# Tonmoy1321/Multimodal-DeepFake-Detection

Hardware: AMD Instinct MI355X
Metric: clips/sec (node) XceptionLSTMV 16x299x299 bf16 train (higher is better)
Workload: dtype bf16; 1 GPU; XceptionLSTMV(hidden=128) unfrozen-backbone train step, 16 clips/GPU x 16 frames x 3x299x299, BCE + clip 1.0 + Adam; global_batch=16, frames=16, size=299, mode=unfrozen, optimizer=clip 1.0 + Adam, xcp FusedAdamClip, parallelism=dp1, execution=eager launches

## Files before the change

include/xcp.h:

```cpp
#ifndef XCP_H_
#define XCP_H_

#ifdef __cplusplus
extern "C" {
#endif

typedef void* xcp_stream_t;

#define XCP_OK 0
#define XCP_EINVAL 1001
#define XCP_EUNSUPPORTED 1002
#define XCP_F32 0
#define XCP_BF16 1
#define XCP_ACT_NONE 0
#define XCP_ACT_RELU 1
#define XCP_ACT_BNRELU 2

int xcp_gemm_nt(int dtype, const void* A, long lda, const void* B, long ldb, void* C, long ldc, int M, int N, int K,
                float* stats, int gmode, int gH, int gW, int gOH, int gOW, int gS, int gC, int tile, xcp_stream_t stream);
int xcp_gemm_nt_stat_rows(int M);

int xcp_gemm_tn_rows_per_split(int dtype, int gmode, int M, int N, int K, int tile);
int xcp_gemm_tn(int dtype, const void* G, long ldg, const void* X, long ldx, float* P, int M, int N, int K, int S,
                int rows_per_split, int gmode, int gH, int gW, int gOH, int gOW, int gS, int gC, int tile,
                xcp_stream_t stream);

int xcp_unit_bwd_rows_per_split(int dtype, int M, int CO, int CI);
int xcp_unit_bwd(int dtype, const void* G, const void* Y, const float* alpha, const float* bcoef, const float* delta,
                 const void* Wt, const void* X, void* dD, float* P, int M, int CO, int CI, int S, int rows_per_split,
                 xcp_stream_t stream);

int xcp_dw_fwd(int dtype, int act, const void* X, void* Y, const float* Wt, const float* scale, const float* shift, int N,
               int H, int W, int C, xcp_stream_t stream);
int xcp_sep_fwd_parts(int dtype, int N, int H, int W, int CIN, int COUT);
int xcp_sep_fwd(int dtype, int act, const void* X, const float* scale, const float* shift, const float* dwt, const void* pw,
                void* D, void* Y, float* part, int N, int H, int W, int CIN, int COUT, xcp_stream_t stream);
int xcp_dw_bwd_chunks(int N, int H, int W, int C);
int xcp_dw_bwd(int dtype, int act, const void* dY, const void* X, const float* Wt, const float* scale, const float* shift,
               const void* dRes, const void* dSkip, int sOH, int sOW, int sS, int skip_pre, void* dX, float* dWpart,
               float* bnpart, const float* bmean, const float* binvstd, int N, int H, int W, int C,
               xcp_stream_t stream);
int xcp_dw_bwd_resbn(int dtype, int act, const void* dY, const void* X, const float* Wt, const float* scale,
                     const float* shift, const void* dRes, void* dX, float* dWpart, float* bnpart, const float* bmean,
                     const float* binvstd, const void* Yb, int N, int H, int W, int C, xcp_stream_t stream);

int xcp_colreduce_f32(const float* in, int S, long L, long ld, float* out, int G, int accumulate, xcp_stream_t stream);
int xcp_colreduce_multi(const long long* jobs, int njobs, xcp_stream_t stream);
int xcp_colreduce_groups(int S, long L);
int xcp_chanred_parts(long rows, int C);
int xcp_row_stats(int dtype, const void* X, long rows, int C, float* part, xcp_stream_t stream);
int xcp_bn_bwd_reduce(int dtype, const void* dZ, const void* Y, const float* mean, const float* invstd,
                      const float* ms, const float* mt, long rows, int C, float* part, xcp_stream_t stream);
int xcp_bn_finalize_part(const float* part, int R, int C, int CP, double count, const float* gamma, const float* beta,
                         float* rmean, float* rvar, float momentum, float eps, float* mean_o, float* invstd_o,
                         float* scale_o, float* shift_o, xcp_stream_t stream);
#define XCP_FIN_ACCUMULATE 1
#define XCP_FIN_NARROW 2
#define XCP_FIN_FROZEN 4
int xcp_bn_bwd_finalize_part(const float* part, int R, int C, int CP, double count, const float* gamma,
                             const float* mean, const float* invstd, float* alpha, float* bcoef, float* delta,
                             float* dgamma, float* dbeta, int flags, xcp_stream_t stream);
int xcp_bn_finalize(const double* part2, int G, int C, int CP, double count, const float* gamma, const float* beta,
                    float* rmean, float* rvar, float momentum, float eps, int train, float* mean, float* invstd,
                    float* scale, float* shift, xcp_stream_t stream);
int xcp_bn_act(int dtype, const void* X, void* Y, const float* scale, const float* shift, int relu, long rows, int C,
               xcp_stream_t stream);
int xcp_bn_act_strided(int dtype, const void* X, void* Y, const float* scale, const float* shift, int relu, int N, int H,
                       int W, int OH, int OW, int S, int C, xcp_stream_t stream);
int xcp_bn_bwd_apply(int dtype, const void* dZ, const void* Y, void* dY, const float* alpha, const float* bcoef,
// ... 102 lines not shown
```

multimodal-deepfake-detection_amd/xcp/_lib.py:

```python
import ctypes
import os

_HERE = os.path.dirname(os.path.abspath(__file__))
LIB_PATH = DEFAULT_LIB_PATH = os.path.join(_HERE, "libxcp.so")
_REPO = os.path.dirname(os.path.dirname(_HERE))
_OVERRIDE = os.environ.get("XCP_LIB_PATH")
if _OVERRIDE:
    _real = os.path.realpath(_OVERRIDE)
    if os.path.commonpath([_real, os.path.realpath(_REPO)]) != os.path.realpath(_REPO):
        raise ImportError(f"XCP_LIB_PATH={_OVERRIDE} is outside the repository ({_REPO}); "
                          "only in-tree A/B builds may replace libxcp.so")
    LIB_PATH = _real
MISSING = []

P = ctypes.c_void_p
I = ctypes.c_int
L = ctypes.c_long
F = ctypes.c_float
D = ctypes.c_double

SIGNATURES = {
    "xcp_gemm_nt": [I, P, L, P, L, P, L, I, I, I, P, I, I, I, I, I, I, I, I, P],
    "xcp_gemm_nt_stat_rows": [I],
    "xcp_gemm_tn_rows_per_split": [I, I, I, I, I, I],
    "xcp_gemm_tn": [I, P, L, P, L, P, I, I, I, I, I, I, I, I, I, I, I, I, I, P],
    "xcp_unit_bwd_rows_per_split": [I, I, I, I],
    "xcp_unit_bwd": [I, P, P, P, P, P, P, P, P, P, I, I, I, I, I, P],
    "xcp_dw_fwd": [I, I, P, P, P, P, P, I, I, I, I, P],
    "xcp_sep_fwd_parts": [I, I, I, I, I, I],
    "xcp_sep_fwd": [I, I, P, P, P, P, P, P, P, P, I, I, I, I, I, P],
    "xcp_dw_bwd_chunks": [I, I, I, I],
    "xcp_dw_bwd": [I, I, P, P, P, P, P, P, P, I, I, I, I, P, P, P, P, P, I, I, I, I, P],
    "xcp_dw_bwd_resbn": [I, I, P, P, P, P, P, P, P, P, P, P, P, P, I, I, I, I, P],
    "xcp_colreduce_f32": [P, I, L, L, P, I, I, P],
    "xcp_colreduce_groups": [I, L],
    "xcp_colreduce_multi": [P, I, P],
    "xcp_chanred_parts": [L, I],
    "xcp_row_stats": [I, P, L, I, P, P],
    "xcp_bn_bwd_reduce": [I, P, P, P, P, P, P, L, I, P, P],
    "xcp_bn_finalize_part": [P, I, I, I, D, P, P, P, P, F, F, P, P, P, P, P],
    "xcp_bn_bwd_finalize_part": [P, I, I, I, D, P, P, P, P, P, P, P, P, I, P],
    "xcp_bn_finalize": [P, I, I, I, D, P, P, P, P, F, F, I, P, P, P, P, P],
    "xcp_bn_act": [I, P, P, P, P, I, L, I, P],
    "xcp_bn_act_strided": [I, P, P, P, P, I, I, I, I, I, I, I, I, P],
    "xcp_bn_bwd_apply": [I, P, P, P, P, P, P, P, P, L, I, P],
    "xcp_relu_bwd": [I, P, P, L, I, P],
    "xcp_tail_fwd": [I, P, P, P, I, P, P, P, P, P, I, I, I, I, P],
    "xcp_maxpool_bwd": [I, P, P, P, I, I, I, I, P],
    "xcp_maxpool_bwd_bnred_parts": [I, I, I, I],
    "xcp_maxpool_bwd_bnred": [I, P, P, P, P, P, P, I, I, I, I, P, P],
    "xcp_avgpool_fwd": [I, P, P, P, P, I, I, I, P],
    "xcp_avgpool_bwd": [I, P, P, P, P, P, I, I, I, P],
    "xcp_conv1_fwd": [I, P, P, P, I, I, I, P],
    "xcp_conv1_fwd_parts": [I, I, I],
    "xcp_conv1_fwd_stats": [I, P, P, P, P, I, I, I, P],
    "xcp_conv1_wgrad_parts": [I, I, I],
    "xcp_conv1_wgrad": [I, P, P, P, I, I, I, P],
    "xcp_conv1_wgrad_fused": [I, I, I],
    "xcp_conv1_wgrad_bn": [I, P, P, P, P, P, P, P, P, P, I, I, I, P],
    "xcp_conv1_dgrad": [I, P, P, P, I, I, I, P],
    "xcp_conv1_dgrad_bn": [I, P, P, P, P, P, P, P, P, P, I, I, I, P],
    "xcp_permute3": [I, P, P, I, I, I, I, I, I, P],
    "xcp_permute3_blocks": [I, I, I, I, I, I, L, L],
    "xcp_permute3_batch": [P, I, I, P],
    "xcp_frames_u8_to_f32": [P, P, P, I, I, I, I, P],
    "xcp_resize_bilinear": [P, P, I, I, I, I, I, P],
    "xcp_frames_prep": [P, P, P, I, I, I, I, I, I, I, I, P],
    "xcp_opt_sumsq": [P, I, P, F, P, P],
    "xcp_opt_adam": [P, I, P, F, F, F, F, F, F, F, P],
    "xcp_opt_adam_dev": [P, I, P, F, D, D, F, F, P, P],
    "xcp_opt_sumsq_amp": [P, I, P, F, P, P, P],
    "xcp_opt_adam_amp": [P, I, P, F, F, F, F, F, F, F, F, P, P, P],
    "xcp_opt_adam_amp_dev": [P, I, P, F, D, D, F, F, F, P, P, P, P],
    "xcp_opt_average": [P, I, P, D, P, P],
    "xcp_conv3x3_parts": [I, I, I, I],
    "xcp_conv3x3": [I, P, P, P, P, I, I, I, P, P, P],
    "xcp_conv3x3_wgrad_parts": [I, I, I],
    "xcp_conv3x3_wgrad": [P, P, P, I, I, I, P, P, P],
    "xcp_arcface_fwd": [P, P, P, P, I, I, I, F, F, P],
    "xcp_arcface_bwd": [P, P, P, P, P, P, I, I, I, F, F, P],
    "xcp_focal_ce": [P, P, P, F, P, P, P, I, I, P],
    "xcp_lstm_needs_whhT": [I, I, I],
    "xcp_lstm_fwd": [P, P, P, P, P, P, P, P, P, P, P, I, I, I, I, P],
    "xcp_lstm_bwd": [P, P, P, P, P, P, P, P, I, I, I, I, P],
    "xcp_lstm_sync_error": [],
    "xcp_lstm_varlen_needs_whhT": [I, I, I],
    "xcp_lstm_fwd_varlen": [P, P, P, P, P, P, P, P, P, P, P, P, I, I, I, I, P],
    "xcp_lstm_bwd_varlen": [P, P, P, P, P, P, P, P, P, I, I, I, I, P],
    "xcp_clock_probe": [P, I, I, P],
    "xcp_stream_copy": [P, P, L, P],
    "xcp_comm_proxy": [P, P, L, I, ctypes.c_longlong, P, P],
    "xcp_stamp": [P, P],
}

SIZE_QUERIES = {"xcp_permute3_blocks", "xcp_sep_fwd_parts", "xcp_gemm_tn_rows_per_split", "xcp_gemm_nt_stat_rows", "xcp_dw_bwd_chunks", "xcp_chanred_parts",
                "xcp_colreduce_groups", "xcp_unit_bwd_rows_per_split",
                "xcp_conv1_wgrad_parts", "xcp_conv1_wgrad_fused", "xcp_conv1_fwd_parts", "xcp_lstm_needs_whhT", "xcp_conv3x3_parts", "xcp_conv3x3_wgrad_parts",
                "xcp_maxpool_bwd_bnred_parts", "xcp_lstm_sync_error", "xcp_lstm_varlen_needs_whhT"}

_lib = None


class XcpError(RuntimeError):
    pass


def load():
    global _lib
    if _lib is not None:
        return _lib
    import torch
    if not os.path.exists(LIB_PATH):
        raise XcpError(f"HIP library {LIB_PATH} is missing; run `python -m xcp.build` (hipcc, gfx950). "
                       "There is no CPU fallback for the product path.")
    lib = ctypes.CDLL(LIB_PATH)
    for name, argtypes in SIGNATURES.items():
        if LIB_PATH != DEFAULT_LIB_PATH and not hasattr(lib, name):
            MISSING.append(name)
            continue
        fn = getattr(lib, name)
        fn.argtypes = argtypes
        fn.restype = ctypes.c_int
    if LIB_PATH != DEFAULT_LIB_PATH:
        import sys
        print(f"xcp: XCP_LIB_PATH override {LIB_PATH}; entry points it lacks: {MISSING or 'none'}",
              file=sys.stderr)
    _lib = lib
    return lib
# ... 14 lines not shown
```

multimodal-deepfake-detection_amd/xcp/csrc/sepfwd.hip:

```cpp
#include "common.h"

namespace {

constexpr int SP_WMAX = 152;
constexpr int SP_WMAX1 = 78;
constexpr int SP_HALF = 80;
constexpr int SP_SEG = 5;
constexpr unsigned SP_OOB = 0x80000000u;
constexpr int SP_REC = 0x7fffffff;
constexpr int SP_DW3 = 0x00020000;

typedef int i32x4 __attribute__((ext_vector_type(4)));
typedef int i32x2 __attribute__((ext_vector_type(2)));
typedef unsigned u32x4 __attribute__((ext_vector_type(4)));
typedef float f2 __attribute__((ext_vector_type(2)));


XCP_DEV u32x4 sp_bload(__amdgpu_buffer_rsrc_t r, int off) {
  u32x4 v;
  asm volatile("buffer_load_dwordx4 %0, %1, %2, 0 offen" : "=v"(v) : "v"(off), "s"(r) : "memory");
  return v;
}

template <int N>
// ... 10 lines not shown
  const bf16* pw;
  bf16* D;
  bf16* Y;
  float* part;
  int N, H, W;
  int nbands, bandH;
};

XCP_DEV void sp_vm_wait(int n) {
  switch (n < 0 ? 0 : n > 63 ? 63 : n) {
#define SP_VMW(k) case k: asm volatile("s_waitcnt vmcnt(" #k ")" ::: "memory"); break;
    SP_VMW(0) SP_VMW(1) SP_VMW(2) SP_VMW(3) SP_VMW(4) SP_VMW(5) SP_VMW(6) SP_VMW(7)
    SP_VMW(8) SP_VMW(9) SP_VMW(10) SP_VMW(11) SP_VMW(12) SP_VMW(13) SP_VMW(14) SP_VMW(15)
    SP_VMW(16) SP_VMW(17) SP_VMW(18) SP_VMW(19) SP_VMW(20) SP_VMW(21) SP_VMW(22) SP_VMW(23)
    SP_VMW(24) SP_VMW(25) SP_VMW(26) SP_VMW(27) SP_VMW(28) SP_VMW(29) SP_VMW(30) SP_VMW(31)
    SP_VMW(32) SP_VMW(33) SP_VMW(34) SP_VMW(35) SP_VMW(36) SP_VMW(37) SP_VMW(38) SP_VMW(39)
#undef SP_VMW
    default: asm volatile("s_waitcnt vmcnt(40)" ::: "memory"); break;
  }
}

XCP_DEV void sp_barrier() {
  asm volatile("s_waitcnt lgkmcnt(0)" ::: "memory");
  __builtin_amdgcn_s_barrier();
  asm volatile("" ::: "memory");
}

XCP_DEV float sp_lo(unsigned u) { return __uint_as_float(u << 16); }
XCP_DEV float sp_hi(unsigned u) { return __uint_as_float(u & 0xffff0000u); }
XCP_DEV unsigned sp_pack(float a, float b) { return pk_bf16(a, b); }

template <int ACT, int CIN, int COUT, int NHALF>
__global__ __launch_bounds__(512) void sep_fwd_kernel(SepArgs a) {
  constexpr int SP_RPX = (NHALF == 2 ? SP_WMAX : SP_WMAX1) + 2;
  constexpr int NB = COUT / 128;
  constexpr int YC = COUT / 8;
  constexpr int S = CIN / 32;
  constexpr int CH = CIN / 8;
  constexpr int PB = CIN * 2;
  constexpr int RB = SP_RPX * PB;
  constexpr int DP = PB + 16;
  constexpr int KL = (SP_RPX * CH + 511) / 512;
  constexpr int KD = (SP_HALF * CH + 511) / 512;
  constexpr int LPS = CIN / 2;
  constexpr int SPW = 64 / LPS;
  constexpr int NPASS = (SP_HALF / SP_SEG) / (8 * SPW);
  constexpr int YP = COUT * 2 + 16;
  constexpr int KY = (SP_HALF * YC + 511) / 512;
  constexpr bool YSHARE = YP == DP;
  constexpr int NST = NHALF * (KD + KY);
  static_assert(NST + KL <= 39, "counted wait exceeds sp_vm_wait's range");
  __shared__ __attribute__((aligned(16))) char rows[3 * RB];
  __shared__ __attribute__((aligned(16))) char dt[SP_HALF * DP];
  __shared__ __attribute__((aligned(16))) char yown[YSHARE ? 16 : SP_HALF * YP];
  char* const yt = YSHARE ? dt : yown;
  __shared__ __attribute__((aligned(16))) float stap[9][CIN];
  __shared__ __attribute__((aligned(16))) float sprm[2][CIN];

  const int tid = threadIdx.x, lane = tid & 63, w = __builtin_amdgcn_readfirstlane(tid >> 6);
  const int fr = lane & 15, fg = lane >> 4;
  const int H = a.H, W = a.W;
  const int nch = (W + 2) * CH;
  const __amdgpu_buffer_rsrc_t rD = __builtin_amdgcn_make_buffer_rsrc(a.D, (short)0, SP_REC, SP_DW3);
  const __amdgpu_buffer_rsrc_t rY = __builtin_amdgcn_make_buffer_rsrc(a.Y, (short)0, SP_REC, SP_DW3);

  bf16x8 wf[NB][S];
#pragma unroll
  for (int j = 0; j < NB; ++j)
#pragma unroll
    for (int s = 0; s < S; ++s)
      wf[j][s] = *reinterpret_cast<const bf16x8*>(a.pw + (long)((w + 8 * j) * 16 + fr) * CIN + s * 32 + fg * 8);
  for (int c = tid; c < 9 * CIN; c += 512) stap[c / CIN][c % CIN] = a.dwt[c];
  for (int c = tid; c < CIN; c += 512) {
    sprm[0][c] = ACT == ACT_BNRELU ? a.scale[c] : 1.f;
    sprm[1][c] = ACT == ACT_BNRELU ? a.shift[c] : 0.f;
  }
  __syncthreads();
  const int ch = 2 * (lane % LPS);
  const int q = tid % CH;
  f2 s1[4], s2[4];
#pragma unroll
  for (int r = 0; r < 4; ++r) s1[r] = s2[r] = f2{0.f, 0.f};

  u32x4 rga[KL], rgb[KL];
  int loff[KL];
#pragma unroll
  for (int k = 0; k < KL; ++k) {
    const int c = tid + 512 * k;
    const int px = c / CH;
    loff[k] = c < nch && px >= 1 && px <= W ? ((px - 1) * CIN + q * 8) * 2 : (int)SP_OOB;
  }
  auto load_row = [&](u32x4 (&rg)[KL], int n, int hh) {
    const bool rok = hh >= 0 && hh < H;
    const __amdgpu_buffer_rsrc_t rs = __builtin_amdgcn_make_buffer_rsrc(
        const_cast<bf16*>(a.X + ((long)n * H + (rok ? hh : 0)) * W * CIN), (short)0, rok ? SP_REC : 0, SP_DW3);
#pragma unroll
    for (int k = 0; k < KL; ++k) rg[k] = sp_bload(rs, loff[k]);
  };
  auto store_row = [&](u32x4 (&rg)[KL], int hh) {
    sp_fence(rg);
    char* slot = rows + ((hh + 3) % 3) * RB;
#pragma unroll
    for (int k = 0; k < KL; ++k) {
      const int c = tid + 512 * k;
      if (c >= nch) continue;
      const int px = c / CH;
      uint4 u = make_uint4(rg[k][0], rg[k][1], rg[k][2], rg[k][3]);
      if constexpr (ACT != ACT_NONE) {
        if (hh >= 0 && hh < H && px >= 1 && px <= W) {
          unsigned v[4] = {u.x, u.y, u.z, u.w};
#pragma unroll
          for (int e = 0; e < 4; ++e) {
            f2 x = f2{sp_lo(v[e]), sp_hi(v[e])};
            if constexpr (ACT == ACT_BNRELU)
              x = __builtin_elementwise_fma(x, *reinterpret_cast<const f2*>(&sprm[0][q * 8 + 2 * e]),
                                            *reinterpret_cast<const f2*>(&sprm[1][q * 8 + 2 * e]));
            x = __builtin_elementwise_max(x, f2{0.f, 0.f});
            v[e] = sp_pack(x[0], x[1]);
          }
          u = make_uint4(v[0], v[1], v[2], v[3]);
        }
      }
      *reinterpret_cast<uint4*>(slot + px * PB + q * 16) = u;
    }
  };

  const int tiles = a.N * a.nbands;
  for (int tile = xcd_remap(blockIdx.x, gridDim.x); tile < tiles; tile += gridDim.x) {
    const int n = tile / a.nbands, band = tile % a.nbands;
    const int r0 = band * a.bandH, r1 = min(H, r0 + a.bandH);
    sp_barrier();
    for (int hh = r0 - 1; hh <= r0 + 1; ++hh) {
      load_row(rga, n, hh);
      sp_vm_wait(0);
      store_row(rga, hh);
    }
    load_row(rga, n, r0 + 2);
    load_row(rgb, n, r0 + 3);
    sp_barrier();
    auto row = [&](int h, u32x4 (&rg)[KL]) {
      const long prow = ((long)n * H + h) * W;
      const char* rw0 = rows + ((h + 2) % 3) * RB;
      const char* rw1 = rows + ((h + 3) % 3) * RB;
      const char* rw2 = rows + ((h + 4) % 3) * RB;
#pragma unroll
      for (int hf = 0; hf < NHALF; ++hf) {
        f32x4 acc[5][NB];
#pragma unroll
        for (int b = 0; b < 5; ++b)
#pragma unroll
          for (int j = 0; j < NB; ++j) acc[b][j] = f32x4{0.f, 0.f, 0.f, 0.f};
#pragma unroll 1
        for (int p = 0; p < NPASS; ++p) {
          const int seg = p * 8 * SPW + w * SPW + lane / LPS;
          const int xl = seg * SP_SEG;
          const int x0 = hf * SP_HALF + xl;
          f2 tp[9];
#pragma unroll
          for (int t = 0; t < 9; ++t) tp[t] = *reinterpret_cast<const f2*>(&stap[t][ch]);
          f2 win[3][SP_SEG + 2];
#pragma unroll
          for (int k = 0; k < SP_SEG + 2; ++k) {
            const int off = min(x0 + k, W + 1) * PB + ch * 2;
            const unsigned u0 = *reinterpret_cast<const unsigned*>(rw0 + off);
            const unsigned u1 = *reinterpret_cast<const unsigned*>(rw1 + off);
            const unsigned u2 = *reinterpret_cast<const unsigned*>(rw2 + off);
            win[0][k] = f2{sp_lo(u0), sp_hi(u0)};
            win[1][k] = f2{sp_lo(u1), sp_hi(u1)};
            win[2][k] = f2{sp_lo(u2), sp_hi(u2)};
          }
#pragma unroll
          for (int jj = 0; jj < SP_SEG; ++jj) {
            f2 d = f2{0.f, 0.f};
#pragma unroll
            for (int ky = 0; ky < 3; ++ky)
#pragma unroll
              for (int kx = 0; kx < 3; ++kx) d = __builtin_elementwise_fma(win[ky][jj + kx], tp[ky * 3 + kx], d);
            *reinterpret_cast<unsigned*>(dt + (xl + jj) * DP + ch * 2) = x0 + jj < W ? sp_pack(d[0], d[1]) : 0u;
          }
        }
        sp_barrier();
#pragma unroll
        for (int b = 0; b < 5; ++b)
#pragma unroll
          for (int s = 0; s < S; ++s) {
            const bf16x8 ad = *reinterpret_cast<const bf16x8*>(dt + (b * 16 + fr) * DP + (s * 32 + fg * 8) * 2);
#pragma unroll
            for (int j = 0; j < NB; ++j) acc[b][j] = __builtin_amdgcn_mfma_f32_16x16x32_bf16(wf[j][s], ad, acc[b][j], 0, 0, 0);
          }
#pragma unroll
        for (int k = 0; k < KD; ++k) {
          const int c = tid + 512 * k;
          const int pl = min(c / CH, SP_HALF - 1), qq = c % CH;
          const int px = hf * SP_HALF + pl;
          const bool ok = c < SP_HALF * CH && px < W;
          const uint4 v = *reinterpret_cast<const uint4*>(dt + pl * DP + qq * 16);
          const unsigned off = ok ? (unsigned)(((prow + px) * CIN + qq * 8) * 2) : SP_OOB;
          __builtin_amdgcn_raw_buffer_store_b128(__builtin_bit_cast(i32x4, v), rD, (int)off, 0, 0);
        }
        if constexpr (YSHARE) sp_barrier();
#pragma unroll
        for (int b = 0; b < 5; ++b)
#pragma unroll
          for (int j = 0; j < NB; ++j)
            *reinterpret_cast<uint2*>(yt + (b * 16 + fr) * YP + ((w + 8 * j) * 16 + 4 * fg) * 2) =
                make_uint2(sp_pack(acc[b][j][0], acc[b][j][1]), sp_pack(acc[b][j][2], acc[b][j][3]));
        sp_barrier();
#pragma unroll
        for (int k = 0; k < KY; ++k) {
          const int c = tid + 512 * k;
          const int pl = min(c / YC, SP_HALF - 1), qq = c % YC;
          const int px = hf * SP_HALF + pl;
          const bool ok = c < SP_HALF * YC && px < W;
          const uint4 v = *reinterpret_cast<const uint4*>(yt + pl * YP + qq * 16);
          const unsigned off = ok ? (unsigned)(((prow + px) * COUT + qq * 8) * 2) : SP_OOB;
          __builtin_amdgcn_raw_buffer_store_b128(__builtin_bit_cast(i32x4, v), rY, (int)off, 0, 0);
          if (ok) {
            const unsigned u4[4] = {v.x, v.y, v.z, v.w};
#pragma unroll
            for (int r = 0; r < 4; ++r) {
              const f2 y = f2{sp_lo(u4[r]), sp_hi(u4[r])};
              s1[r] += y;
              s2[r] = __builtin_elementwise_fma(y, y, s2[r]);
            }
          }
        }
        sp_barrier();
      }
      sp_vm_wait(NST + KL);
      store_row(rg, h + 2);
      load_row(rg, n, h + 4);
      sp_barrier();
    };
    for (int h = r0; h < r1; h += 2) {
      row(h, rga);
      if (h + 1 < r1) row(h + 1, rgb);
    }
    sp_vm_wait(0);
  }
  sp_vm_wait(0);
  if (a.part) {
    float t[2][8];
#pragma unroll
    for (int r = 0; r < 4; ++r)
#pragma unroll
      for (int e = 0; e < 2; ++e) {
        t[0][2 * r + e] = s1[r][e];
        t[1][2 * r + e] = s2[r][e];
      }
#pragma unroll
    for (int m = 0; m < 2; ++m)
#pragma unroll
      for (int e = 0; e < 8; ++e) {
        if constexpr (YC == 16) t[m][e] += __shfl_xor(t[m][e], 16, 64);
        t[m][e] += __shfl_xor(t[m][e], 32, 64);
      }
    sp_barrier();
// ... 3 lines not shown
      for (int m = 0; m < 2; ++m)
#pragma unroll
        for (int e = 0; e < 8; ++e) red[(w * 2 + m) * COUT + lane * 8 + e] = t[m][e];
    sp_barrier();
    for (int i = tid; i < 2 * COUT; i += 512) {
      float v = 0.f;
#pragma unroll
      for (int ww = 0; ww < 8; ++ww) v += red[ww * 2 * COUT + i];
      a.part[(long)blockIdx.x * 2 * COUT + i] = v;
    }
  }
}

int sp_cus() {
  static const int v = [] {
    int dev = 0, n = 0;
    if (hipGetDevice(&dev) != hipSuccess || hipDeviceGetAttribute(&n, hipDeviceAttributeMultiprocessorCount, dev) != hipSuccess)
      n = 0;
    return n > 0 ? n : 256;
  }();
  return v;
}

void sp_bands(int N, int H, int& nb, int& bandH) {
  const int cus = sp_cus();
  nb = N >= cus ? 1 : (cus + N - 1) / N;
  const int maxb = H >= 16 ? H / 8 : 1;
  if (nb > maxb) nb = maxb;
  if (nb < 1) nb = 1;
  bandH = (H + nb - 1) / nb;
  nb = (H + bandH - 1) / bandH;
}

}

extern "C" {

int xcp_sep_fwd_parts(int dtype, int N, int H, int W, int CIN, int COUT) {
  const bool shape = (COUT == 128 && (CIN == 64 || CIN == 128) && W <= SP_WMAX) ||
                     (COUT == 256 && CIN == 128 && W <= SP_WMAX1);
  if (dtype != XCP_BF16 || !shape || W < 1 || N <= 0 || H <= 0) return 0;
  const long pix = (long)N * H * W;
  if (pix * CIN * 2 > 0x7fffffffL || pix * COUT * 2 > 0x7fffffffL) return 0;
  int nb, bh;
  sp_bands(N, H, nb, bh);
  const long tiles = (long)N * nb;
  return (int)(tiles < sp_cus() ? tiles : sp_cus());
}

int xcp_sep_fwd(int dtype, int act, const void* X, const float* scale, const float* shift, const float* dwt, const void* pw,
                void* D, void* Y, float* part, int N, int H, int W, int CIN, int COUT, hipStream_t stream) {
  const int grid = xcp_sep_fwd_parts(dtype, N, H, W, CIN, COUT);
  if (grid <= 0) return XCP_EUNSUPPORTED;
  if (act < ACT_NONE || act > ACT_BNRELU || (act == ACT_BNRELU && (!scale || !shift))) return XCP_EINVAL;
  SepArgs a{(const bf16*)X, scale, shift, dwt, (const bf16*)pw, (bf16*)D, (bf16*)Y, part, N, H, W, 1, H};
  sp_bands(N, H, a.nbands, a.bandH);
#define SP_LAUNCH(A, C, O, NH) hipLaunchKernelGGL((sep_fwd_kernel<A, C, O, NH>), dim3(grid), dim3(512), 0, stream, a)
#define SP_ACTS(C, O, NH)                          \
  if (act == ACT_NONE) SP_LAUNCH(ACT_NONE, C, O, NH); \
  else if (act == ACT_RELU) SP_LAUNCH(ACT_RELU, C, O, NH); \
  else SP_LAUNCH(ACT_BNRELU, C, O, NH);
  if (COUT == 256) {
    SP_ACTS(128, 256, 1)
  } else if (CIN == 64) {
    SP_ACTS(64, 128, 2)
  } else {
    SP_ACTS(128, 128, 2)
  }
#undef SP_ACTS
#undef SP_LAUNCH
  return (int)hipGetLastError();
}

}
```

multimodal-deepfake-detection_amd/xcp/engine.py:

```python
import contextlib
import os
import math

import torch
import torch.nn as nn

from . import ops
from .ops import ACT_BNRELU, ACT_NONE, ACT_RELU


def _bn_ref(m):
    return {"weight": m.weight, "bias": m.bias, "running_mean": m.running_mean, "running_var": m.running_var,
            "eps": m.eps, "momentum": m.momentum, "track": m.track_running_stats, "module": m}


class _Unit:

    def __init__(self, sep, bn, relu, name, bn_name):
        self.sep, self.bn, self.relu, self.name, self.bn_name = sep, bn, relu, name, bn_name
        self.cin = sep.conv1.in_channels
        self.cout = sep.pointwise.out_channels
        if sep.conv1.kernel_size != (3, 3) or sep.conv1.stride != (1, 1) or sep.conv1.padding != (1, 1):
            raise NotImplementedError("xcp engine supports the Xception 3x3/s1/p1 separable convs only")
        if sep.conv1.bias is not None or sep.pointwise.bias is not None:
# ... 34 lines not shown
        if self.pool and self.skip is None:
            raise NotImplementedError("xcp engine: a pooled block needs a conv skip")
        if self.skip is not None and self.stride != (2 if self.pool else 1):
            raise NotImplementedError("xcp engine: skip stride must match the pooling")
        self.cin = self.units[0].cin
        self.cout = self.units[-1].cout


class Stats:
    __slots__ = ("mean", "invstd", "scale", "shift")

    def __init__(self, C, dev):
        buf = torch.empty(4 * C, device=dev, dtype=torch.float32)
        self.mean, self.invstd, self.scale, self.shift = buf[:C], buf[C:2 * C], buf[2 * C:3 * C], buf[3 * C:]

    def __getitem__(self, k):
        return getattr(self, k)


WGRAD_SIDE_STREAM = os.environ.get("XCP_WGRAD_STREAM", "1") != "0"
FUSED_UNIT_BWD = os.environ.get("XCP_FUSED_UNIT_BWD", "1") != "0"
STEM_FUSED = os.environ.get("XCP_STEM_FUSED", "1") != "0"
RESBN = os.environ.get("XCP_RESBN", "0") == "1"
STEM_WGRAD_SIDE = WGRAD_SIDE_STREAM and os.environ.get("XCP_STEM_WGRAD_SIDE", "1") != "0"
SIDE_PRIO_LOW = os.environ.get("XCP_SIDE_PRIO", "") == "low"
STEM_BN1_FIRST = os.environ.get("XCP_STEM_BN1_FIRST", "1") != "0"
CONV1_BN_FUSED = os.environ.get("XCP_CONV1_BN_FUSED", "1") != "0"
STEM_WGRAD_EARLY = os.environ.get("XCP_STEM_WGRAD_EARLY", "1") != "0"
STEM_FIN_NARROW = os.environ.get("XCP_STEM_FIN_NARROW", "1") != "0"
CONV1_STATS_FUSED = os.environ.get("XCP_CONV1_STATS_FUSED", "1") != "0"
DW_REDUCE_SIDE = WGRAD_SIDE_STREAM and os.environ.get("XCP_DW_REDUCE_SIDE", "1") != "0"
REDUCE_BATCH = os.environ.get("XCP_REDUCE_BATCH", "1") != "0"
SEP_FUSED = os.environ.get("XCP_SEP_FUSED", "1") != "0"
SEP_MIN_W = {128: 0, 256: 0} if os.environ.get("XCP_SEP_NARROW", "0") == "1" else {128: 120, 256: 64}
CONV2_ACT_ON_LOAD = os.environ.get("XCP_CONV2_ACTIN", "1") != "0"
WGRAD_FIRST = os.environ.get("XCP_WGRAD_FIRST", "0") == "1"
WGRAD_DEFER = os.environ.get("XCP_WGRAD_DEFER", "0") == "1"
SKIP_WGRAD_LATE = os.environ.get("XCP_SKIP_WGRAD_LATE", "0") == "1"
NT_TILE = int(os.environ.get("XCP_NT_TILE", "4" if os.environ.get("XCP_NT_ONESHOT", "0") == "1" else "0"))
_pad = os.environ.get("XCP_PAD_728", "736")
PAD_PITCH = {} if _pad == "0" else {728: int(_pad)}
if PAD_PITCH and (PAD_PITCH[728] < 728 or PAD_PITCH[728] % 8):
    raise ValueError("XCP_PAD_728 must be 0 or a multiple of 8 >= 728")


def pc(c):
    return PAD_PITCH.get(c, c)


class XceptionEngine:
    def __init__(self, model, dtype=torch.bfloat16):
        if dtype not in (torch.float32, torch.bfloat16):
            raise ValueError("xcp engine dtype must be float32 (parity) or bfloat16")
        self.model = model
        self.dtype = dtype
        self.blocks = [_Block(getattr(model, f"block{i}"), f"block{i}") for i in range(1, 13)]
        self.exit_units = [_Unit(model.conv3, model.bn3, False, "conv3", "bn3"),
                           _Unit(model.conv4, model.bn4, True, "conv4", "bn4")]
        c1, c2 = model.conv1, model.conv2
        if (c1.in_channels, c1.out_channels, c1.kernel_size, c1.stride, c1.padding) != (3, 32, (3, 3), (2, 2), (0, 0)):
            raise NotImplementedError("xcp engine: Xception stem conv1 must be 3->32 3x3 s2 p0")
        if (c2.in_channels, c2.out_channels, c2.kernel_size, c2.stride, c2.padding) != (32, 64, (3, 3), (1, 1), (0, 0)):
            raise NotImplementedError("xcp engine: Xception stem conv2 must be 32->64 3x3 s1 p0")
        self.bn_named = [(n, m) for n, m in model.named_modules() if isinstance(m, nn.BatchNorm2d)]
        self.bn_modules = [m for _, m in self.bn_named]
        self._pack_key = None
# ... 195 lines not shown
            H, W, rest = OH2, OW2, self.blocks
        for b in rest:
            xc, H, W, bs = self._block_fwd(b, xc, N, H, W, pk, train)
            S["blocks"].append(bs)
        M = N * H * W
        ex = []
        src, act, sc, sh = xc, ACT_NONE, None, None
        for u in self.exit_units:
            d = self._empty(M * pc(u.cin))
            ops.dw_fwd(act, src, d, pk[u.name + ".dw"], sc, sh, N, H, W, pc(u.cin))
            y, st = self._pw(d, pk[u.name + ".pw"], M, u.cout, u.cin, train, u.bn)
            ex.append({"src": src, "act": act, "sc": sc, "sh": sh, "d": d, "y": y, "st": st})
            src, act, sc, sh = y, ACT_BNRELU, st.scale, st.shift
        feats = torch.empty(N, 2048, device=self.device, dtype=torch.float32)
        last = ex[-1]
        ops.avgpool_fwd(last["y"], last["st"].scale, last["st"].shift, feats, N, H * W, 2048)
        S.update(exit=ex, xH=H, xW=W, x12=xc)
        if train:
            nbt = [b.num_batches_tracked for b in self.bn_modules if b.num_batches_tracked is not None]
            if nbt:
                torch._foreach_add_(nbt, 1)
        return feats, S

    def _block_fwd(self, b, x_in, N, H, W, pk, train, pre_bn=None, skip_x=None):
        if pre_bn is not None and (b.skip is None or b.stride == 1 or b.units[0].relu):
            raise ValueError("pre_bn: only a block without a leading ReLU and with a strided skip conv")
        M = N * H * W
        units = []
        src, act, sc, sh = x_in, (ACT_RELU if b.units[0].relu else ACT_NONE), None, None
        if pre_bn is not None:
            act, sc, sh = ACT_BNRELU, pre_bn.scale, pre_bn.shift
        for u in b.units:
            d = self._empty(M * pc(u.cin))
            R = (ops.sep_fwd_parts(self.dtype, N, H, W, u.cin, u.cout)
                 if SEP_FUSED and train and pc(u.cin) == u.cin and pc(u.cout) == u.cout
                 and W >= SEP_MIN_W.get(u.cout, 1 << 30) else 0)
            if R > 0:
                y = self._empty(M * u.cout)
                part = self._empty(R * 2 * u.cout, torch.float32)
                ops.sep_fwd(act, src, sc, sh, pk[u.name + ".dw"], pk[u.name + ".pw"], d, y, part, N, H, W, u.cin, u.cout)
                st = self._bn_stats(part, R, u.cout, M, u.bn, True)
            else:
                ops.dw_fwd(act, src, d, pk[u.name + ".dw"], sc, sh, N, H, W, pc(u.cin))
                y, st = self._pw(d, pk[u.name + ".pw"], M, u.cout, u.cin, train, u.bn)
            units.append({"src": src, "act": act, "sc": sc, "sh": sh, "d": d, "y": y, "st": st})
            src, act, sc, sh = y, ACT_BNRELU, st.scale, st.shift
        if b.pool or b.stride != 1:
            OH, OW = (H - 1) // b.stride + 1, (W - 1) // b.stride + 1
        else:
            OH, OW = H, W
        Ms = N * OH * OW
        ys = sks = None
        if b.skip is not None and skip_x is not None:
            ys, sks = self._pw(skip_x, pk[b.name + ".skip"], Ms, b.cout, b.cin, train, b.skipbn, lda=pc(b.cin))
        elif b.skip is not None:
            ys, sks = self._pw(x_in, pk[b.name + ".skip"], Ms, b.cout, b.cin, train, b.skipbn, lda=pc(b.cin),
                               gather=(1, H, W, OH, OW, b.stride, 0) if b.stride != 1 else (0, 0, 0, 0, 0, 1, 0))
        out = self._empty(Ms * pc(b.cout))
        amax = torch.empty(Ms * pc(b.cout), device=self.device, dtype=torch.uint8) if b.pool else None
        st = units[-1]["st"]
        ops.tail_fwd(units[-1]["y"], st.scale, st.shift, b.pool, ys if ys is not None else x_in,
                     sks.scale if sks is not None else None, sks.shift if sks is not None else None, out, amax, N, H, W,
                     pc(b.cout))
        bs = {"x_in": x_in, "units": units, "ys": ys, "sks": sks, "amax": amax, "H": H, "W": W, "OH": OH, "OW": OW,
              "pre_bn": pre_bn, "skip_x": skip_x}
        return out, OH, OW, bs

    INPUT = "<frames>"

    def backward(self, S, dfeat, out=None, notify=None, need=None, input_grad=False):
        with ops.device_guard(dfeat):
            return self._backward(S, dfeat, out, notify, need, input_grad)

# ... 288 lines not shown
```

multimodal-deepfake-detection_amd/xcp/ops.py:

```python
import torch

from . import _lib

F32, BF16 = 0, 1
ACT_NONE, ACT_RELU, ACT_BNRELU = 0, 1, 2
DT = {torch.float32: F32, torch.bfloat16: BF16}


def _p(t):
    return 0 if t is None else t.data_ptr()


def stream():
    return torch.cuda.current_stream().cuda_stream


def device_guard(t):
    return torch.cuda.device(t.device)


class KernelTimer:

    def __init__(self, classes):
        self.classes = classes
# ... 121 lines not shown
                arr = (ctypes.c_longlong * len(vals))(*vals)
                _lib.call("xcp_colreduce_multi", ctypes.addressof(arr), len(chunk), stream())
        self.jobs = []


def weight_grad(G, X, M, N, K, out, gather=(0, 0, 0, 0, 0, 1, 0), ldg=None, ldx=None, tile=0, accumulate=False,
                batch=None):
    rps = _lib.call("xcp_gemm_tn_rows_per_split", DT[G.dtype], gather[0], M, N, K, tile)
    S = (M + rps - 1) // rps
    P = torch.empty(S * N * K, device=G.device, dtype=torch.float32)
    gemm_tn(G, X, P, M, N, K, S, rps, ldg=ldg, ldx=ldx, gather=gather, tile=tile)
    if batch is not None:
        batch.add(P, S, N * K, out, accumulate)
    else:
        reduce_slabs(P, S, N * K, out, accumulate)


def dw_fwd(act, X, Y, Wt, scale, shift, N, H, W, C):
    with _timed("dw_fwd", {"N": N, "H": H, "W": W, "C": C}):
        _lib.call("xcp_dw_fwd", DT[X.dtype], act, _p(X), _p(Y), _p(Wt), _p(scale), _p(shift), N, H, W, C, stream())


def sep_fwd_parts(dtype, N, H, W, cin, cout):
    return _lib.call("xcp_sep_fwd_parts", DT[dtype], N, H, W, cin, cout)


def sep_fwd(act, X, scale, shift, dwt, pw, D, Y, part, N, H, W, cin, cout):
    check_gpu(X, D, Y)
    with _timed("sep_fwd", {"N": N, "H": H, "W": W, "C": cin, "CO": cout}):
        _lib.call("xcp_sep_fwd", DT[X.dtype], act, _p(X), _p(scale), _p(shift), _p(dwt), _p(pw), _p(D), _p(Y), _p(part),
                  N, H, W, cin, cout, stream())


def dw_bwd(act, dY, X, Wt, scale, shift, dX, dW_out, N, H, W, C, dRes=None, dSkip=None, skip_geom=(0, 0, 1),
           bn_stats=None, accumulate=False, Cw=None, skip_pre=False, reduce_stream=None, keep=None, batch=None,
           res_bn_input=None):
    P = _lib.call("xcp_dw_bwd_chunks", N, H, W, C)
    part = torch.empty(P * C * 9, device=dY.device, dtype=torch.float32)
    bnpart = None
    if bn_stats is not None:
        bnpart = torch.empty(P * 2 * C, device=dY.device, dtype=torch.float32)
    if res_bn_input is not None:
        if dRes is None or dSkip is not None or bn_stats is None:
            raise ValueError("xcp.dw_bwd: res_bn_input needs dRes, no dSkip and the BN's bn_stats")
        _lib.call("xcp_dw_bwd_resbn", DT[dY.dtype], act, _p(dY), _p(X), _p(Wt), _p(scale), _p(shift), _p(dRes),
                  _p(dX), _p(part), _p(bnpart), _p(bn_stats["mean"]), _p(bn_stats["invstd"]), _p(res_bn_input),
                  N, H, W, C, stream())
    else:
        _lib.call("xcp_dw_bwd", DT[dY.dtype], act, _p(dY), _p(X), _p(Wt), _p(scale), _p(shift), _p(dRes), _p(dSkip),
                  skip_geom[0], skip_geom[1], skip_geom[2], int(skip_pre), _p(dX), _p(part), _p(bnpart),
                  _p(bn_stats["mean"]) if bn_stats is not None else 0,
                  _p(bn_stats["invstd"]) if bn_stats is not None else 0, N, H, W, C, stream())
    if dW_out is None:
        pass
    elif batch is not None:
        batch.add(part, P, (Cw or C) * 9, dW_out, accumulate, ld=C * 9)
        if keep is not None:
            keep.append(part)
    elif reduce_stream is None:
        reduce_slabs(part, P, (Cw or C) * 9, dW_out, accumulate, ld=C * 9)
    else:
        reduce_stream.wait_stream(torch.cuda.current_stream(dY.device))
        with torch.cuda.stream(reduce_stream):
            reduce_slabs(part, P, (Cw or C) * 9, dW_out, accumulate, ld=C * 9)
        if keep is not None:
            keep.append(part)
# ... 330 lines not shown
```

Measured before the change: 441.9 clips/s.

## Extend fused depthwise+pointwise separable forward kernel to 256->256 channel units

Adds a CIN=256/COUT=256 variant of the fused separable-conv forward kernel. It keeps the depthwise taps and BN scale/shift in registers instead of LDS so the wider tile fits in shared memory, and it narrows the row tile. The engine now routes 256->256 units (block2/3 style, act on input) to it instead of separate dw_fwd plus pointwise GEMM. The aim is to avoid writing and re-reading the depthwise output between kernels and to save a launch, at the cost of higher register pressure and smaller tiles.

```diff
diff --git a/include/xcp.h b/include/xcp.h
--- a/include/xcp.h
+++ b/include/xcp.h
@@ -35,6 +35,9 @@
 int xcp_sep_fwd_parts(int dtype, int N, int H, int W, int CIN, int COUT);
 int xcp_sep_fwd(int dtype, int act, const void* X, const float* scale, const float* shift, const float* dwt, const void* pw,
                 void* D, void* Y, float* part, int N, int H, int W, int CIN, int COUT, xcp_stream_t stream);
+int xcp_sep_fwd256_parts(int dtype, int N, int H, int W);
+int xcp_sep_fwd256(int dtype, int act, const void* X, const float* scale, const float* shift, const float* dwt, const void* pw,
+                   void* D, void* Y, float* part, int N, int H, int W, xcp_stream_t stream);
 int xcp_dw_bwd_chunks(int N, int H, int W, int C);
 int xcp_dw_bwd(int dtype, int act, const void* dY, const void* X, const float* Wt, const float* scale, const float* shift,
                const void* dRes, const void* dSkip, int sOH, int sOW, int sS, int skip_pre, void* dX, float* dWpart,
diff --git a/multimodal-deepfake-detection_amd/xcp/_lib.py b/multimodal-deepfake-detection_amd/xcp/_lib.py
--- a/multimodal-deepfake-detection_amd/xcp/_lib.py
+++ b/multimodal-deepfake-detection_amd/xcp/_lib.py
@@ -29,6 +29,8 @@
     "xcp_dw_fwd": [I, I, P, P, P, P, P, I, I, I, I, P],
     "xcp_sep_fwd_parts": [I, I, I, I, I, I],
     "xcp_sep_fwd": [I, I, P, P, P, P, P, P, P, P, I, I, I, I, I, P],
+    "xcp_sep_fwd256_parts": [I, I, I, I],
+    "xcp_sep_fwd256": [I, I, P, P, P, P, P, P, P, P, I, I, I, P],
     "xcp_dw_bwd_chunks": [I, I, I, I],
     "xcp_dw_bwd": [I, I, P, P, P, P, P, P, P, I, I, I, I, P, P, P, P, P, I, I, I, I, P],
     "xcp_dw_bwd_resbn": [I, I, P, P, P, P, P, P, P, P, P, P, P, P, I, I, I, I, P],
@@ -93,7 +95,7 @@
     "xcp_stamp": [P, P],
 }
 
-SIZE_QUERIES = {"xcp_permute3_blocks", "xcp_sep_fwd_parts", "xcp_gemm_tn_rows_per_split", "xcp_gemm_nt_stat_rows", "xcp_dw_bwd_chunks", "xcp_chanred_parts",
+SIZE_QUERIES = {"xcp_permute3_blocks", "xcp_sep_fwd_parts", "xcp_sep_fwd256_parts", "xcp_gemm_tn_rows_per_split", "xcp_gemm_nt_stat_rows", "xcp_dw_bwd_chunks", "xcp_chanred_parts",
                 "xcp_colreduce_groups", "xcp_unit_bwd_rows_per_split",
                 "xcp_conv1_wgrad_parts", "xcp_conv1_wgrad_fused", "xcp_conv1_fwd_parts", "xcp_lstm_needs_whhT", "xcp_conv3x3_parts", "xcp_conv3x3_wgrad_parts",
                 "xcp_maxpool_bwd_bnred_parts", "xcp_lstm_sync_error", "xcp_lstm_varlen_needs_whhT"}
diff --git a/multimodal-deepfake-detection_amd/xcp/csrc/sepfwd.hip b/multimodal-deepfake-detection_amd/xcp/csrc/sepfwd.hip
--- a/multimodal-deepfake-detection_amd/xcp/csrc/sepfwd.hip
+++ b/multimodal-deepfake-detection_amd/xcp/csrc/sepfwd.hip
@@ -66,35 +66,40 @@
 
 template <int ACT, int CIN, int COUT, int NHALF>
 __global__ __launch_bounds__(512) void sep_fwd_kernel(SepArgs a) {
+  constexpr bool WIDE = CIN == 256;
+  static_assert(!WIDE || NHALF == 1, "CIN = 256: the one-half form only");
   constexpr int SP_RPX = (NHALF == 2 ? SP_WMAX : SP_WMAX1) + 2;
+  constexpr int TPX = WIDE ? SP_WMAX1 : SP_HALF;
   constexpr int NB = COUT / 128;
   constexpr int YC = COUT / 8;
   constexpr int S = CIN / 32;
   constexpr int CH = CIN / 8;
   constexpr int PB = CIN * 2;
-  constexpr int RB = SP_RPX * PB;
+  constexpr int RB = (WIDE ? SP_RPX - 1 : SP_RPX) * PB;
   constexpr int DP = PB + 16;
-  constexpr int KL = (SP_RPX * CH + 511) / 512;
-  constexpr int KD = (SP_HALF * CH + 511) / 512;
+  constexpr int KL = ((WIDE ? SP_WMAX1 : SP_RPX) * CH + 511) / 512;
+  constexpr int KD = (TPX * CH + 511) / 512;
   constexpr int LPS = CIN / 2;
-  constexpr int SPW = 64 / LPS;
-  constexpr int NPASS = (SP_HALF / SP_SEG) / (8 * SPW);
+  constexpr int WPS = WIDE ? LPS / 64 : 1;
+  constexpr int SPW = WIDE ? 1 : 64 / LPS;
+  constexpr int NPASS = (SP_HALF / SP_SEG) / (8 / WPS * SPW);
   constexpr int YP = COUT * 2 + 16;
-  constexpr int KY = (SP_HALF * YC + 511) / 512;
+  constexpr int KY = (TPX * YC + 511) / 512;
   constexpr bool YSHARE = YP == DP;
   constexpr int NST = NHALF * (KD + KY);
   static_assert(NST + KL <= 39, "counted wait exceeds sp_vm_wait's range");
-  __shared__ __attribute__((aligned(16))) char rows[3 * RB];
-  __shared__ __attribute__((aligned(16))) char dt[SP_HALF * DP];
+  static_assert(!WIDE || YSHARE, "CIN = 256: no room for a Y tile of its own");
+  __shared__ __attribute__((aligned(16))) char rows[3 * RB + (WIDE ? PB : 0)];
+  __shared__ __attribute__((aligned(16))) char dt[TPX * DP];
   __shared__ __attribute__((aligned(16))) char yown[YSHARE ? 16 : SP_HALF * YP];
   char* const yt = YSHARE ? dt : yown;
-  __shared__ __attribute__((aligned(16))) float stap[9][CIN];
-  __shared__ __attribute__((aligned(16))) float sprm[2][CIN];
+  __shared__ __attribute__((aligned(16))) float stap[WIDE ? 1 : 9][WIDE ? 4 : CIN];
+  __shared__ __attribute__((aligned(16))) float sprm[WIDE ? 1 : 2][WIDE ? 4 : CIN];
 
   const int tid = threadIdx.x, lane = tid & 63, w = __builtin_amdgcn_readfirstlane(tid >> 6);
   const int fr = lane & 15, fg = lane >> 4;
   const int H = a.H, W = a.W;
-  const int nch = (W + 2) * CH;
+  const int nch = (WIDE ? W : W + 2) * CH;
   const __amdgpu_buffer_rsrc_t rD = __builtin_amdgcn_make_buffer_rsrc(a.D, (short)0, SP_REC, SP_DW3);
   const __amdgpu_buffer_rsrc_t rY = __builtin_amdgcn_make_buffer_rsrc(a.Y, (short)0, SP_REC, SP_DW3);
 
@@ -104,14 +109,36 @@
 #pragma unroll
     for (int s = 0; s < S; ++s)
       wf[j][s] = *reinterpret_cast<const bf16x8*>(a.pw + (long)((w + 8 * j) * 16 + fr) * CIN + s * 32 + fg * 8);
-  for (int c = tid; c < 9 * CIN; c += 512) stap[c / CIN][c % CIN] = a.dwt[c];
-  for (int c = tid; c < CIN; c += 512) {
-    sprm[0][c] = ACT == ACT_BNRELU ? a.scale[c] : 1.f;
-    sprm[1][c] = ACT == ACT_BNRELU ? a.shift[c] : 0.f;
+  const int ch = WIDE ? 2 * (lane + 64 * (w % WPS)) : 2 * (lane % LPS);
+  const int q = tid % CH;
+  f2 rtap[9], rprm[2][4];
+  if constexpr (WIDE) {
+#pragma unroll
+    for (int t = 0; t < 9; ++t) rtap[t] = *reinterpret_cast<const f2*>(a.dwt + t * CIN + ch);
+#pragma unroll
+    for (int e = 0; e < 4; ++e) {
+      rprm[0][e] = ACT == ACT_BNRELU ? *reinterpret_cast<const f2*>(a.scale + q * 8 + 2 * e) : f2{1.f, 1.f};
+      rprm[1][e] = ACT == ACT_BNRELU ? *reinterpret_cast<const f2*>(a.shift + q * 8 + 2 * e) : f2{0.f, 0.f};
+    }
+    for (int c = tid; c < 6 * CH; c += 512)
+      *reinterpret_cast<uint4*>(rows + (c / (2 * CH)) * RB + ((c / CH) & 1 ? W + 1 : 0) * PB + (c % CH) * 16) =
+          make_uint4(0u, 0u, 0u, 0u);
+#pragma unroll
+    for (int t = 0; t < 9; ++t) asm volatile("" : "+v"(rtap[t]));
+#pragma unroll
+    for (int e = 0; e < 4; ++e) asm volatile("" : "+v"(rprm[0][e]), "+v"(rprm[1][e]));
+#pragma unroll
+    for (int j = 0; j < NB; ++j)
+#pragma unroll
+      for (int s = 0; s < S; ++s) asm volatile("" : "+v"(wf[j][s]));
+  } else {
+    for (int c = tid; c < 9 * CIN; c += 512) stap[c / CIN][c % CIN] = a.dwt[c];
+    for (int c = tid; c < CIN; c += 512) {
+      sprm[0][c] = ACT == ACT_BNRELU ? a.scale[c] : 1.f;
+      sprm[1][c] = ACT == ACT_BNRELU ? a.shift[c] : 0.f;
+    }
   }
   __syncthreads();
-  const int ch = 2 * (lane % LPS);
-  const int q = tid % CH;
   f2 s1[4], s2[4];
 #pragma unroll
   for (int r = 0; r < 4; ++r) s1[r] = s2[r] = f2{0.f, 0.f};
@@ -121,7 +148,7 @@
 #pragma unroll
   for (int k = 0; k < KL; ++k) {
     const int c = tid + 512 * k;
-    const int px = c / CH;
+    const int px = WIDE ? c / CH + 1 : c / CH;
     loff[k] = c < nch && px >= 1 && px <= W ? ((px - 1) * CIN + q * 8) * 2 : (int)SP_OOB;
   }
   auto load_row = [&](u32x4 (&rg)[KL], int n, int hh) {
@@ -138,7 +165,7 @@
     for (int k = 0; k < KL; ++k) {
       const int c = tid + 512 * k;
       if (c >= nch) continue;
-      const int px = c / CH;
+      const int px = WIDE ? c / CH + 1 : c / CH;
       uint4 u = make_uint4(rg[k][0], rg[k][1], rg[k][2], rg[k][3]);
       if constexpr (ACT != ACT_NONE) {
         if (hh >= 0 && hh < H && px >= 1 && px <= W) {
@@ -146,9 +173,13 @@
 #pragma unroll
           for (int e = 0; e < 4; ++e) {
             f2 x = f2{sp_lo(v[e]), sp_hi(v[e])};
-            if constexpr (ACT == ACT_BNRELU)
-              x = __builtin_elementwise_fma(x, *reinterpret_cast<const f2*>(&sprm[0][q * 8 + 2 * e]),
-                                            *reinterpret_cast<const f2*>(&sprm[1][q * 8 + 2 * e]));
+            if constexpr (ACT == ACT_BNRELU) {
+              if constexpr (WIDE)
+                x = __builtin_elementwise_fma(x, rprm[0][e], rprm[1][e]);
+              else
+                x = __builtin_elementwise_fma(x, *reinterpret_cast<const f2*>(&sprm[0][q * 8 + 2 * e]),
+                                              *reinterpret_cast<const f2*>(&sprm[1][q * 8 + 2 * e]));
+            }
             x = __builtin_elementwise_max(x, f2{0.f, 0.f});
             v[e] = sp_pack(x[0], x[1]);
           }
@@ -186,12 +217,12 @@
           for (int j = 0; j < NB; ++j) acc[b][j] = f32x4{0.f, 0.f, 0.f, 0.f};
 #pragma unroll 1
         for (int p = 0; p < NPASS; ++p) {
-          const int seg = p * 8 * SPW + w * SPW + lane / LPS;
+          const int seg = WIDE ? p * (8 / WPS) + w / WPS : p * 8 * SPW + w * SPW + lane / LPS;
           const int xl = seg * SP_SEG;
           const int x0 = hf * SP_HALF + xl;
           f2 tp[9];
 #pragma unroll
-          for (int t = 0; t < 9; ++t) tp[t] = *reinterpret_cast<const f2*>(&stap[t][ch]);
+          for (int t = 0; t < 9; ++t) tp[t] = WIDE ? rtap[t] : *reinterpret_cast<const f2*>(&stap[t][ch]);
           f2 win[3][SP_SEG + 2];
 #pragma unroll
           for (int k = 0; k < SP_SEG + 2; ++k) {
@@ -210,7 +241,8 @@
             for (int ky = 0; ky < 3; ++ky)
 #pragma unroll
               for (int kx = 0; kx < 3; ++kx) d = __builtin_elementwise_fma(win[ky][jj + kx], tp[ky * 3 + kx], d);
-            *reinterpret_cast<unsigned*>(dt + (xl + jj) * DP + ch * 2) = x0 + jj < W ? sp_pack(d[0], d[1]) : 0u;
+            if (!WIDE || xl + jj < TPX)
+              *reinterpret_cast<unsigned*>(dt + (xl + jj) * DP + ch * 2) = x0 + jj < W ? sp_pack(d[0], d[1]) : 0u;
           }
         }
         sp_barrier();
@@ -218,16 +250,16 @@
         for (int b = 0; b < 5; ++b)
 #pragma unroll
           for (int s = 0; s < S; ++s) {
-            const bf16x8 ad = *reinterpret_cast<const bf16x8*>(dt + (b * 16 + fr) * DP + (s * 32 + fg * 8) * 2);
+            const bf16x8 ad = *reinterpret_cast<const bf16x8*>(dt + min(b * 16 + fr, TPX - 1) * DP + (s * 32 + fg * 8) * 2);
 #pragma unroll
             for (int j = 0; j < NB; ++j) acc[b][j] = __builtin_amdgcn_mfma_f32_16x16x32_bf16(wf[j][s], ad, acc[b][j], 0, 0, 0);
           }
 #pragma unroll
         for (int k = 0; k < KD; ++k) {
           const int c = tid + 512 * k;
-          const int pl = min(c / CH, SP_HALF - 1), qq = c % CH;
+          const int pl = min(c / CH, TPX - 1), qq = c % CH;
           const int px = hf * SP_HALF + pl;
-          const bool ok = c < SP_HALF * CH && px < W;
+          const bool ok = c < TPX * CH && px < W;
           const uint4 v = *reinterpret_cast<const uint4*>(dt + pl * DP + qq * 16);
           const unsigned off = ok ? (unsigned)(((prow + px) * CIN + qq * 8) * 2) : SP_OOB;
           __builtin_amdgcn_raw_buffer_store_b128(__builtin_bit_cast(i32x4, v), rD, (int)off, 0, 0);
@@ -237,15 +269,19 @@
         for (int b = 0; b < 5; ++b)
 #pragma unroll
           for (int j = 0; j < NB; ++j)
-            *reinterpret_cast<uint2*>(yt + (b * 16 + fr) * YP + ((w + 8 * j) * 16 + 4 * fg) * 2) =
-                make_uint2(sp_pack(acc[b][j][0], acc[b][j][1]), sp_pack(acc[b][j][2], acc[b][j][3]));
+            if (b * 16 + fr < TPX)
+              *reinterpret_cast<uint2*>(yt + (b * 16 + fr) * YP + ((w + 8 * j) * 16 + 4 * fg) * 2) =
+                  make_uint2(sp_pack(acc[b][j][0], acc[b][j][1]), sp_pack(acc[b][j][2], acc[b][j][3]));
         sp_barrier();
+        f2 rs1[4], rs2[4];
+#pragma unroll
+        for (int r = 0; r < 4; ++r) rs1[r] = rs2[r] = f2{0.f, 0.f};
 #pragma unroll
         for (int k = 0; k < KY; ++k) {
           const int c = tid + 512 * k;
-          const int pl = min(c / YC, SP_HALF - 1), qq = c % YC;
+          const int pl = min(c / YC, TPX - 1), qq = c % YC;
           const int px = hf * SP_HALF + pl;
-          const bool ok = c < SP_HALF * YC && px < W;
+          const bool ok = c < TPX * YC && px < W;
           const uint4 v = *reinterpret_cast<const uint4*>(yt + pl * YP + qq * 16);
           const unsigned off = ok ? (unsigned)(((prow + px) * COUT + qq * 8) * 2) : SP_OOB;
           __builtin_amdgcn_raw_buffer_store_b128(__builtin_bit_cast(i32x4, v), rY, (int)off, 0, 0);
@@ -254,9 +290,21 @@
 #pragma unroll
             for (int r = 0; r < 4; ++r) {
               const f2 y = f2{sp_lo(u4[r]), sp_hi(u4[r])};
-              s1[r] += y;
-              s2[r] = __builtin_elementwise_fma(y, y, s2[r]);
+              if constexpr (WIDE) {
+                rs1[r] += y;
+                rs2[r] = __builtin_elementwise_fma(y, y, rs2[r]);
+              } else {
+                s1[r] += y;
+                s2[r] = __builtin_elementwise_fma(y, y, s2[r]);
+              }
             }
+          }
+        }
+        if constexpr (WIDE) {
+#pragma unroll
+          for (int r = 0; r < 4; ++r) {
+            s1[r] += rs1[r];
+            s2[r] += rs2[r];
           }
         }
         sp_barrier();
@@ -326,13 +374,7 @@
   nb = (H + bandH - 1) / bandH;
 }
 
-}
-
-extern "C" {
-
-int xcp_sep_fwd_parts(int dtype, int N, int H, int W, int CIN, int COUT) {
-  const bool shape = (COUT == 128 && (CIN == 64 || CIN == 128) && W <= SP_WMAX) ||
-                     (COUT == 256 && CIN == 128 && W <= SP_WMAX1);
+int sp_grid(bool shape, int dtype, int N, int H, int W, int CIN, int COUT) {
   if (dtype != XCP_BF16 || !shape || W < 1 || N <= 0 || H <= 0) return 0;
   const long pix = (long)N * H * W;
   if (pix * CIN * 2 > 0x7fffffffL || pix * COUT * 2 > 0x7fffffffL) return 0;
@@ -342,9 +384,38 @@
   return (int)(tiles < sp_cus() ? tiles : sp_cus());
 }
 
+int sp_launch(int grid, int act, const void* X, const float* scale, const float* shift, const float* dwt, const void* pw,
+              void* D, void* Y, float* part, int N, int H, int W, int CIN, int COUT, hipStream_t stream);
+
+}
+
+extern "C" {
+
+int xcp_sep_fwd_parts(int dtype, int N, int H, int W, int CIN, int COUT) {
+  const bool shape = (COUT == 128 && (CIN == 64 || CIN == 128) && W <= SP_WMAX) ||
+                     (COUT == 256 && CIN == 128 && W <= SP_WMAX1);
+  return sp_grid(shape, dtype, N, H, W, CIN, COUT);
+}
+
 int xcp_sep_fwd(int dtype, int act, const void* X, const float* scale, const float* shift, const float* dwt, const void* pw,
                 void* D, void* Y, float* part, int N, int H, int W, int CIN, int COUT, hipStream_t stream) {
-  const int grid = xcp_sep_fwd_parts(dtype, N, H, W, CIN, COUT);
+  return sp_launch(xcp_sep_fwd_parts(dtype, N, H, W, CIN, COUT), act, X, scale, shift, dwt, pw, D, Y, part, N, H, W, CIN, COUT,
+                   stream);
+}
+
+int xcp_sep_fwd256_parts(int dtype, int N, int H, int W) { return sp_grid(W <= SP_WMAX1, dtype, N, H, W, 256, 256); }
+
+int xcp_sep_fwd256(int dtype, int act, const void* X, const float* scale, const float* shift, const float* dwt, const void* pw,
+                   void* D, void* Y, float* part, int N, int H, int W, hipStream_t stream) {
+  return sp_launch(xcp_sep_fwd256_parts(dtype, N, H, W), act, X, scale, shift, dwt, pw, D, Y, part, N, H, W, 256, 256, stream);
+}
+
+}
+
+namespace {
+
+int sp_launch(int grid, int act, const void* X, const float* scale, const float* shift, const float* dwt, const void* pw,
+              void* D, void* Y, float* part, int N, int H, int W, int CIN, int COUT, hipStream_t stream) {
   if (grid <= 0) return XCP_EUNSUPPORTED;
   if (act < ACT_NONE || act > ACT_BNRELU || (act == ACT_BNRELU && (!scale || !shift))) return XCP_EINVAL;
   SepArgs a{(const bf16*)X, scale, shift, dwt, (const bf16*)pw, (bf16*)D, (bf16*)Y, part, N, H, W, 1, H};
@@ -354,7 +425,11 @@
   if (act == ACT_NONE) SP_LAUNCH(ACT_NONE, C, O, NH); \
   else if (act == ACT_RELU) SP_LAUNCH(ACT_RELU, C, O, NH); \
   else SP_LAUNCH(ACT_BNRELU, C, O, NH);
-  if (COUT == 256) {
+  if (CIN == 256) {
+    if (act == ACT_NONE) return XCP_EUNSUPPORTED;
+    if (act == ACT_RELU) SP_LAUNCH(ACT_RELU, 256, 256, 1);
+    else SP_LAUNCH(ACT_BNRELU, 256, 256, 1);
+  } else if (COUT == 256) {
     SP_ACTS(128, 256, 1)
   } else if (CIN == 64) {
     SP_ACTS(64, 128, 2)
diff --git a/multimodal-deepfake-detection_amd/xcp/engine.py b/multimodal-deepfake-detection_amd/xcp/engine.py
--- a/multimodal-deepfake-detection_amd/xcp/engine.py
+++ b/multimodal-deepfake-detection_amd/xcp/engine.py
@@ -90,6 +90,7 @@
 DW_REDUCE_SIDE = WGRAD_SIDE_STREAM and os.environ.get("XCP_DW_REDUCE_SIDE", "1") != "0"
 REDUCE_BATCH = os.environ.get("XCP_REDUCE_BATCH", "1") != "0"
 SEP_FUSED = os.environ.get("XCP_SEP_FUSED", "1") != "0"
+SEP_FUSED_256 = SEP_FUSED and os.environ.get("XCP_SEP_FUSED_256", "1") != "0"
 SEP_MIN_W = {128: 0, 256: 0} if os.environ.get("XCP_SEP_NARROW", "0") == "1" else {128: 120, 256: 64}
 CONV2_ACT_ON_LOAD = os.environ.get("XCP_CONV2_ACTIN", "1") != "0"
 WGRAD_FIRST = os.environ.get("XCP_WGRAD_FIRST", "0") == "1"
@@ -351,13 +352,19 @@
             act, sc, sh = ACT_BNRELU, pre_bn.scale, pre_bn.shift
         for u in b.units:
             d = self._empty(M * pc(u.cin))
-            R = (ops.sep_fwd_parts(self.dtype, N, H, W, u.cin, u.cout)
-                 if SEP_FUSED and train and pc(u.cin) == u.cin and pc(u.cout) == u.cout
-                 and W >= SEP_MIN_W.get(u.cout, 1 << 30) else 0)
+            wide = (u.cin, u.cout) == (256, 256)
+            R = 0
+            if (SEP_FUSED_256 if wide else SEP_FUSED) and train and W >= SEP_MIN_W.get(u.cout, 1 << 30) \
+                    and pc(u.cin) == u.cin and pc(u.cout) == u.cout and (not wide or act != ACT_NONE):
+                R = (ops.sep_fwd256_parts(self.dtype, N, H, W) if wide
+                     else ops.sep_fwd_parts(self.dtype, N, H, W, u.cin, u.cout))
             if R > 0:
                 y = self._empty(M * u.cout)
                 part = self._empty(R * 2 * u.cout, torch.float32)
-                ops.sep_fwd(act, src, sc, sh, pk[u.name + ".dw"], pk[u.name + ".pw"], d, y, part, N, H, W, u.cin, u.cout)
+                if wide:
+                    ops.sep_fwd256(act, src, sc, sh, pk[u.name + ".dw"], pk[u.name + ".pw"], d, y, part, N, H, W)
+                else:
+                    ops.sep_fwd(act, src, sc, sh, pk[u.name + ".dw"], pk[u.name + ".pw"], d, y, part, N, H, W, u.cin, u.cout)
                 st = self._bn_stats(part, R, u.cout, M, u.bn, True)
             else:
                 ops.dw_fwd(act, src, d, pk[u.name + ".dw"], sc, sh, N, H, W, pc(u.cin))
diff --git a/multimodal-deepfake-detection_amd/xcp/ops.py b/multimodal-deepfake-detection_amd/xcp/ops.py
--- a/multimodal-deepfake-detection_amd/xcp/ops.py
+++ b/multimodal-deepfake-detection_amd/xcp/ops.py
@@ -177,6 +177,17 @@
                   N, H, W, cin, cout, stream())
 
 
+def sep_fwd256_parts(dtype, N, H, W):
+    return _lib.call("xcp_sep_fwd256_parts", DT[dtype], N, H, W)
+
+
+def sep_fwd256(act, X, scale, shift, dwt, pw, D, Y, part, N, H, W):
+    check_gpu(X, D, Y)
+    with _timed("sep_fwd", {"N": N, "H": H, "W": W, "C": 256, "CO": 256}):
+        _lib.call("xcp_sep_fwd256", DT[X.dtype], act, _p(X), _p(scale), _p(shift), _p(dwt), _p(pw), _p(D), _p(Y), _p(part),
+                  N, H, W, stream())
+
+
 def dw_bwd(act, dY, X, Wt, scale, shift, dX, dW_out, N, H, W, C, dRes=None, dSkip=None, skip_geom=(0, 0, 1),
            bn_stats=None, accumulate=False, Cw=None, skip_pre=False, reduce_stream=None, keep=None, batch=None,
            res_bn_input=None):
```

Result: no change. 443.7 clips/s, median of 6 (+0.4%).
